# szemenyeim/RoboCupVision

Measured on AMD Instinct MI355X. Metric: training images/sec, ROBO-UNet 640x480 bs=32/GPU, higher is better.
Workload: dtype f32; 1 GPU; robo_unet_640x480_bs32; per_gpu_batch=32, global_batch=32, height=480, width=640, step=fwd+CE/argmax+bwd+L1+Adam (train.py:43-74), parallelism=dp1, launch=eager (one rcv_run per pass)

## Files before the change

include/rcv.h:

```cpp
#ifndef RCV_H
#define RCV_H

#include <stddef.h>
#include <stdint.h>

#ifdef __cplusplus
extern "C" {
#endif

#define RCV_VERSION 100

#define RCV_OK            0
#define RCV_E_ARG        -1
#define RCV_E_HIP        -2
#define RCV_E_UNSUPPORTED -3

typedef struct rcv_handle rcv_handle;

int  rcv_create(int device, rcv_handle** out);
int  rcv_create_planner(int num_cus, rcv_handle** out);
int  rcv_destroy(rcv_handle* h);
const char* rcv_last_error(void);
int  rcv_version(void);
int  rcv_num_cus(const rcv_handle* h);
// ... 29 lines not shown
  RCV_OP_SGD         = 27,
  RCV_OP_NOP         = 28,
  RCV_OP_WGRAD_REDUCE_BATCH = 29,
  RCV_OP_POOL_CLS_FWD = 30,
  RCV_OP_POOL_CLS_BWD = 31,
  RCV_OP_OBJECT_MATCH = 32,
  RCV_OP_LP_TAIL_FWD = 33,
  RCV_OP_LP_TAIL_BWD = 34,
  RCV_OP_LP_BATCH = 35,
  RCV_OP_BATCH_PREP = 36,
  RCV_OP_CLS_LABEL = 37,
  RCV_OP_FRAME_PREP = 38,
  RCV_OP_BNN_STAGE_FWD = 39,
  RCV_OP_BNN_STAGE_BWD = 40,
  RCV_OP_BNN_HEAD_FWD = 41,
  RCV_OP_BNN_HEAD_BWD = 42
};

enum {
  RCV_LOAD_PLAIN    = 0,
  RCV_LOAD_AFFINE   = 1,
  RCV_LOAD_GRAD_ENC = 2,
  RCV_LOAD_GRAD_DEC = 3,
  RCV_LOAD_NCHW     = 4,
  RCV_LOAD_AFFINE_RELU = 5
};

enum {
  RCV_STATS_NONE   = 0,
  RCV_STATS_FWD    = 1,
  RCV_STATS_BWD_ENC= 2,
// ... 173 lines not shown
```

robocupvision_amd/_lib.py:

```python
from __future__ import annotations

import ctypes as C
import os
import threading

_HERE = os.path.dirname(os.path.abspath(__file__))
LIB_PATH = os.environ.get("RCV_LIBRARY") or os.path.join(_HERE, "librcv.so")

RCV_I_N, RCV_I_H, RCV_I_W, RCV_I_CIN, RCV_I_COUT, RCV_I_HO, RCV_I_WO, RCV_I_STRIDE, RCV_I_DIL, \
    RCV_I_INMODE, RCV_I_INMODE2, RCV_I_STATS, RCV_I_NPART, RCV_I_NSPLIT, RCV_I_COUNT, RCV_I_AUX0, RCV_I_AUX1 = range(17)
RCV_I__N = 20
(RCV_P_IN, RCV_P_IN_AUX, RCV_P_IN_C, RCV_P_W, RCV_P_BIAS, RCV_P_OUT, RCV_P_RESID, RCV_P_EPI_AUX, RCV_P_EPI_C,
 RCV_P_PART, RCV_P_IN2, RCV_P_IN2_AUX, RCV_P_IN2_C, RCV_P_X0, RCV_P_X1, RCV_P_X2, RCV_P_X3, RCV_P_X4, RCV_P_X5) = range(19)
RCV_P__N = 20

(OP_CONV, OP_TCONV, OP_WGRAD, OP_WGRAD_REDUCE, OP_PACK, OP_BN_FINALIZE, OP_BN_EVAL, OP_BN_BWD, OP_COMBINE, OP_CLS_FWD,
 OP_CLS_BWD, OP_CE_FWD, OP_CE_BWD, OP_POOL_FWD, OP_POOL_BWD, OP_ADAM_L1, OP_MEMSET, OP_CONV1X1, OP_ADD_SLICE,
 OP_MATERIALIZE, OP_BWD_STATS, OP_CONFUSION, OP_DICE_FWD, OP_DICE_BWD, OP_NHWC_TO_NCHW, OP_NCHW_TO_NHWC, OP_SGD, OP_NOP,
 OP_WGRAD_REDUCE_BATCH, OP_POOL_CLS_FWD, OP_POOL_CLS_BWD) = range(1, 32)
OP_OBJECT_MATCH = 32
OP_LP_TAIL_FWD, OP_LP_TAIL_BWD, OP_LP_BATCH = 33, 34, 35
OP_BATCH_PREP = 36
OP_CLS_LABEL = 37
OP_FRAME_PREP = 38
OP_BNN_STAGE_FWD, OP_BNN_STAGE_BWD, OP_BNN_HEAD_FWD, OP_BNN_HEAD_BWD = 39, 40, 41, 42
CLS_LABEL_FEATURES, CLS_LABEL_LOGITS, CLS_LABEL_CLASSMAP = range(3)

LOAD_PLAIN, LOAD_AFFINE, LOAD_GRAD_ENC, LOAD_GRAD_DEC, LOAD_NCHW, LOAD_AFFINE_RELU = range(6)
STATS_NONE, STATS_FWD, STATS_BWD_ENC, STATS_BWD_DEC = range(4)
F_BIAS, F_RELU, F_RESID, F_OUT_NCHW, F_FLIP, F_TRANSPOSED_SRC, F_ARGMAX, F_TRAINING, F_CONCAT = 1, 2, 4, 8, 16, 32, 64, 128, 256
F_FUSED_UP = 512
F_FUSED_CE = 1024
F_SIDE_STREAM = 1 << 16
F_MFMA_FP32 = 1 << 17


class RcvOp(C.Structure):
    _fields_ = [("kind", C.c_int32), ("flags", C.c_uint32), ("i", C.c_int32 * RCV_I__N), ("f", C.c_float * 8),
                ("p", C.c_void_p * RCV_P__N)]

# ... 161 lines not shown
```

robocupvision_amd/csrc/small_kernels.hip:

```cpp
#include "rcv_internal.h"
#include "cls_common.h"

__device__ __forceinline__ float wave_sum(float v) {
#pragma unroll
  for (int sh = 32; sh >= 1; sh >>= 1) v += __shfl_xor(v, sh);
  return v;
}
__device__ __forceinline__ double wave_sum_d(double v) {
#pragma unroll
  for (int sh = 32; sh >= 1; sh >>= 1) v += __shfl_xor(v, sh);
  return v;
}

__global__ void pack_kernel(const rcv_pack_job* __restrict__ jobs) {
  const rcv_pack_job jb = jobs[blockIdx.y];
  const int per_tap = jb.rows_pad * jb.cols_pad;
  if (jb.merged == 2) {
    const int rows = jb.rows_from_d1 ? jb.D1 : jb.D0;
    const int cols = jb.rows_from_d1 ? jb.D0 : jb.D1;
    for (int e = blockIdx.x * blockDim.x + threadIdx.x; e < per_tap; e += gridDim.x * blockDim.x) {
      const int row = e / jb.cols_pad, col = e - row * jb.cols_pad;
      float g[3][3];
      const bool ok = row < rows && col < cols;
      const int d0 = jb.rows_from_d1 ? col : row, d1 = jb.rows_from_d1 ? row : col;
// ... 185 lines not shown
    v.x = fmaxf(fmaf(a.x, s.x, h.x), 0.f); v.y = fmaxf(fmaf(a.y, s.y, h.y), 0.f);
    v.z = fmaxf(fmaf(a.z, s.z, h.z), 0.f); v.w = fmaxf(fmaf(a.w, s.w, h.w), 0.f);
    float4 b = sld4(r + e * 4);
    if (mode2 != RCV_LOAD_PLAIN) {
      const float4 s2 = sld4(rc + ch), h2 = sld4(rc + C + ch);
      b.x = fmaf(b.x, s2.x, h2.x); b.y = fmaf(b.y, s2.y, h2.y); b.z = fmaf(b.z, s2.z, h2.z); b.w = fmaf(b.w, s2.w, h2.w);
      if (mode2 == RCV_LOAD_AFFINE_RELU) { b.x = fmaxf(b.x, 0.f); b.y = fmaxf(b.y, 0.f); b.z = fmaxf(b.z, 0.f); b.w = fmaxf(b.w, 0.f); }
    }
    sst4(out + pix * 2 * C + ch, v);
    sst4(out + pix * 2 * C + C + ch, b);
  }
}

#define CE_MAX_C 8

template <int CIN, bool FUSED, bool CE>
__global__ void cls_fwd_kernel(const float* __restrict__ x, const float* __restrict__ w, const float* __restrict__ bias,
                               float* __restrict__ out, int N, int HW, int COUT, const float* __restrict__ tc,
                               const float* __restrict__ r, const float* __restrict__ rc, int mode2,
                               const int64_t* __restrict__ target, const float* __restrict__ cw, float* __restrict__ part,
                               uint8_t* __restrict__ argmax, int rch) {
  __shared__ float ws[CLS_MAX_OUT * CIN + CLS_MAX_OUT];
  __shared__ double sh[3][4];
  for (int e = threadIdx.x; e < COUT * CIN; e += blockDim.x) ws[e] = w[e];
  for (int e = threadIdx.x; e < COUT; e += blockDim.x) ws[CLS_MAX_OUT * CIN + e] = bias ? bias[e] : 0.f;
  __syncthreads();
  double a_nll = 0.0, a_w = 0.0, a_ok = 0.0;
  const size_t total = (size_t)N * HW;
  for (size_t p = (size_t)blockIdx.x * blockDim.x + threadIdx.x; p < total; p += (size_t)gridDim.x * blockDim.x) {
    float v[CIN];
    cls_load_up<CIN, FUSED>(v, x, tc, r, rc, mode2, p, rch);
    const size_t n = p / HW, hw = p % HW;
    float lg[CLS_MAX_OUT];
#pragma unroll
    for (int c = 0; c < CLS_MAX_OUT; ++c) {
      if (c < COUT) {
        float u = ws[CLS_MAX_OUT * CIN + c];
#pragma unroll
        for (int k = 0; k < CIN; ++k) u = fmaf(v[k], ws[c * CIN + k], u);
        __builtin_nontemporal_store(u, out + (n * COUT + c) * HW + hw);
        lg[c] = u;
      }
    }
    if (CE) {
      float mx = -INFINITY;
      int am = 0;
#pragma unroll
      for (int c = 0; c < CLS_MAX_OUT; ++c) if (c < COUT && lg[c] > mx) { mx = lg[c]; am = c; }
      float se = 0.f;
#pragma unroll
      for (int c = 0; c < CLS_MAX_OUT; ++c) if (c < COUT) se += expf(lg[c] - mx);
      const int tg = (int)target[p];
      float vt = 0.f;
#pragma unroll
      for (int c = 0; c < CLS_MAX_OUT; ++c) if (c == tg && c < COUT) vt = lg[c];
      const float wt = (unsigned)tg < (unsigned)COUT ? (cw ? cw[tg] : 1.f) : 0.f;
      const float nll = (mx - vt) + logf(se);
      a_nll += (double)(wt * nll);
      a_w += (double)wt;
      a_ok += (am == tg) ? 1.0 : 0.0;
      if (argmax) argmax[p] = (uint8_t)am;
    }
  }
  if (CE) {
    a_nll = wave_sum_d(a_nll); a_w = wave_sum_d(a_w); a_ok = wave_sum_d(a_ok);
    const int wv = threadIdx.x >> 6;
    if ((threadIdx.x & 63) == 0) { sh[0][wv] = a_nll; sh[1][wv] = a_w; sh[2][wv] = a_ok; }
    __syncthreads();
    if (threadIdx.x < 3) {
      double t = 0.0;
      for (int i = 0; i < (int)(blockDim.x >> 6); ++i) t += sh[threadIdx.x][i];
      part[(size_t)blockIdx.x * 3 + threadIdx.x] = (float)t;
    }
  }
}

template <bool FUSED>
__global__ __launch_bounds__(256) void cls_fwd16_kernel(const float* __restrict__ x, const float* __restrict__ w, const float* __restrict__ bias,
                                                        float* __restrict__ out, int N, int HW, int COUT, const float* __restrict__ tc,
                                                        const float* __restrict__ r, const float* __restrict__ rc, int mode2, int rch) {
  constexpr int CIN = 16;
  __shared__ float ws[CLS_MAX_OUT * CIN + CLS_MAX_OUT];
  for (int e = threadIdx.x; e < CLS_MAX_OUT * CIN; e += blockDim.x) ws[e] = e < COUT * CIN ? w[e] : 0.f;
  for (int e = threadIdx.x; e < CLS_MAX_OUT; e += blockDim.x) ws[CLS_MAX_OUT * CIN + e] = (bias && e < COUT) ? bias[e] : 0.f;
  __syncthreads();
  const int q = threadIdx.x & 3;
  float4 s = make_float4(1.f, 1.f, 1.f, 1.f), h = make_float4(0.f, 0.f, 0.f, 0.f), s2 = s, h2 = h;
  if (FUSED) {
// ... 20 lines not shown
#pragma unroll
    for (int c = 0; c < CLS_MAX_OUT; ++c) {
      const float* wc = ws + c * CIN + 4 * q;
      float u = fmaf(a.x, wc[0], fmaf(a.y, wc[1], fmaf(a.z, wc[2], a.w * wc[3])));
      u += __shfl_xor(u, 1);
      u += __shfl_xor(u, 2);
      lg[c] = u + ws[CLS_MAX_OUT * CIN + c];
    }
    const size_t n = p / HW, hw = p % HW;
#pragma unroll
    for (int c = 0; c < CLS_MAX_OUT; ++c)
      if ((c & 3) == q && c < COUT) out[(n * COUT + c) * HW + hw] = lg[c];
  }
}

template <int CIN, int COUT, bool FUSED, bool CE>
__global__ __launch_bounds__(256, (CIN == 8 ? 2 : 1)) void cls_bwd_kernel(const float* __restrict__ up, const float* __restrict__ dl, const float* __restrict__ w,
                               float* __restrict__ dup, const float* __restrict__ t, const float* __restrict__ tc,
                               float* __restrict__ stat_part, float* __restrict__ w_part, int N, int HW, int stats,
                               const float* __restrict__ r, const float* __restrict__ rc, int mode2,
                               const int64_t* __restrict__ target, const float* __restrict__ cw, const float* __restrict__ bias,
                               const float* __restrict__ loss_out, const float* __restrict__ grad_out) {
  __shared__ float ws[COUT * CIN];
  __shared__ float red[4][COUT * CIN + COUT + 2 * CIN];
  for (int e = threadIdx.x; e < COUT * CIN; e += blockDim.x) ws[e] = w[e];
  __syncthreads();
  float dw[COUT][CIN], db[COUT], s1[CIN], s2[CIN];
#pragma unroll
  for (int c = 0; c < COUT; ++c) { db[c] = 0.f;
#pragma unroll
    for (int k = 0; k < CIN; ++k) dw[c][k] = 0.f; }
#pragma unroll
  for (int k = 0; k < CIN; ++k) { s1[k] = 0.f; s2[k] = 0.f; }
  const size_t total = (size_t)N * HW;
  const size_t stride = (size_t)gridDim.x * blockDim.x;
  size_t p = (size_t)blockIdx.x * blockDim.x + threadIdx.x;
  ClsRaw<CIN, FUSED> cur;
  int64_t tcur = 0;
  if (p < total) { cls_load_raw<CIN, FUSED>(cur, FUSED ? t : up, r, p); if (CE) tcur = target[p]; }
  for (; p < total; p += stride) {
    const size_t pn = p + stride < total ? p + stride : p;
    ClsRaw<CIN, FUSED> nxt;
    cls_load_raw<CIN, FUSED>(nxt, FUSED ? t : up, r, pn);
    int64_t tnxt = 0;
    if (CE) tnxt = target[pn];
    const size_t n = p / HW, hw = p % HW;
    float g[COUT], u[CIN], d[CIN];
    cls_form_up<CIN, FUSED>(u, cur, tc, rc, mode2);
    if (CE) {
      float mx = -INFINITY;
#pragma unroll
      for (int c = 0; c < COUT; ++c) {
        float lgc = bias ? bias[c] : 0.f;
#pragma unroll
        for (int k = 0; k < CIN; ++k) lgc = fmaf(u[k], ws[c * CIN + k], lgc);
        g[c] = lgc;
        mx = fmaxf(mx, lgc);
      }
      float se = 0.f;
#pragma unroll
      for (int c = 0; c < COUT; ++c) { g[c] = expf(g[c] - mx); se += g[c]; }
      const int tg = (int)tcur;
      const float kf = (grad_out[0] / loss_out[1]) * ((unsigned)tg < (unsigned)COUT ? (cw ? cw[tg] : 1.f) : 0.f);
      const float inv = 1.f / se;
#pragma unroll
      for (int c = 0; c < COUT; ++c) g[c] = __fmul_rn(kf, fmaf(g[c], inv, c == tg ? -1.f : 0.f));
    } else {
#pragma unroll
      for (int c = 0; c < COUT; ++c) g[c] = dl[(n * COUT + c) * HW + hw];
    }
#pragma unroll
    for (int k = 0; k < CIN; ++k) {
      float acc = 0.f;
#pragma unroll
      for (int c = 0; c < COUT; ++c) acc = fmaf(g[c], ws[c * CIN + k], acc);
      d[k] = acc;
    }
    if (CIN == 8 && (total & 63) == 0) {
      const int lane = threadIdx.x & 63;
      const size_t wave_p0 = p - lane;
#pragma unroll
      for (int sidx = 0; sidx < 2; ++sidx) {
        const int src = sidx * 32 + (lane >> 1);
        float4 lo, hi;
        lo.x = __shfl(d[0], src); lo.y = __shfl(d[1], src); lo.z = __shfl(d[2], src); lo.w = __shfl(d[3], src);
        hi.x = __shfl(d[4], src); hi.y = __shfl(d[5], src); hi.z = __shfl(d[6], src); hi.w = __shfl(d[7], src);
        sst4(dup + (wave_p0 + sidx * 32) * CIN + lane * 4, (lane & 1) ? hi : lo);
      }
    } else {
#pragma unroll
      for (int q = 0; q < CIN / 4; ++q) sst4(dup + p * CIN + 4 * q, make_float4(d[4 * q], d[4 * q + 1], d[4 * q + 2], d[4 * q + 3]));
    }
#pragma unroll
    for (int c = 0; c < COUT; ++c) {
      db[c] += g[c];
#pragma unroll
      for (int k = 0; k < CIN; ++k) dw[c][k] = fmaf(g[c], u[k], dw[c][k]);
    }
    if (stats == RCV_STATS_BWD_DEC) {
#pragma unroll
      for (int q = 0; q < CIN / 4; ++q) {
        const float4 a = FUSED ? cur.a[q] : sld4(t + p * CIN + 4 * q);
// ... 18 lines not shown
    if (lane == 0) red[wv][COUT * CIN + c] = v;
  }
#pragma unroll
  for (int k = 0; k < CIN; ++k) {
    const float v1 = wave_sum(s1[k]), v2 = wave_sum(s2[k]);
    if (lane == 0) { red[wv][COUT * CIN + COUT + k] = v1; red[wv][COUT * CIN + COUT + CIN + k] = v2; }
  }
  __syncthreads();
  const int nw = blockDim.x >> 6;
  for (int e = threadIdx.x; e < COUT * CIN + COUT + 2 * CIN; e += blockDim.x) {
    float v = 0.f;
    for (int i = 0; i < nw; ++i) v += red[i][e];
    if (e < COUT * CIN + COUT) w_part[(size_t)blockIdx.x * (COUT * CIN + COUT) + e] = v;
    else if (stats == RCV_STATS_BWD_DEC) stat_part[(size_t)blockIdx.x * 2 * CIN + (e - COUT * CIN - COUT)] = v;
  }
}

__global__ void rows_reduce_kernel(const float* __restrict__ part, int n_rows, int width, float* __restrict__ out0, int n0,
                                   float* __restrict__ out1) {
  const int e = blockIdx.x;
  double s = 0.0, dummy = 0.0;
  for (int i = threadIdx.x; i < n_rows; i += blockDim.x) s += (double)part[(size_t)i * width + e];
  block_sum2_d(s, dummy);
  if (threadIdx.x == 0) {
    if (e < n0) out0[e] = (float)s;
    else if (out1) out1[e - n0] = (float)s;
  }
}

__global__ void ce_fwd_kernel(const float* __restrict__ logits, const int64_t* __restrict__ target, const float* __restrict__ cw,
                              int N, int C, int HW, float* __restrict__ part, uint8_t* __restrict__ argmax) {
  __shared__ double sh[3][4];
  double a_nll = 0.0, a_w = 0.0, a_ok = 0.0;
  const size_t total = (size_t)N * HW;
  for (size_t p = (size_t)blockIdx.x * blockDim.x + threadIdx.x; p < total; p += (size_t)gridDim.x * blockDim.x) {
    const size_t n = p / HW, hw = p % HW;
    float v[CE_MAX_C];
    float mx = -INFINITY;
    int am = 0;
#pragma unroll
    for (int c = 0; c < CE_MAX_C; ++c) {
      if (c < C) {
// ... 14 lines not shown
    a_w += (double)w;
    a_ok += (am == tg) ? 1.0 : 0.0;
    if (argmax) argmax[p] = (uint8_t)am;
  }
  a_nll = wave_sum_d(a_nll); a_w = wave_sum_d(a_w); a_ok = wave_sum_d(a_ok);
  const int wv = threadIdx.x >> 6;
  if ((threadIdx.x & 63) == 0) { sh[0][wv] = a_nll; sh[1][wv] = a_w; sh[2][wv] = a_ok; }
  __syncthreads();
  if (threadIdx.x < 3) {
    double s = 0.0;
    for (int i = 0; i < (int)(blockDim.x >> 6); ++i) s += sh[threadIdx.x][i];
    part[(size_t)blockIdx.x * 3 + threadIdx.x] = (float)s;
  }
}

__global__ void ce_finalize_kernel(const float* __restrict__ part, int n_part, float* __restrict__ loss_out) {
  __shared__ double sh[3][4];
  double s[3] = {0.0, 0.0, 0.0};
  for (int i = threadIdx.x; i < n_part; i += blockDim.x) {
    s[0] += (double)part[(size_t)i * 3 + 0]; s[1] += (double)part[(size_t)i * 3 + 1]; s[2] += (double)part[(size_t)i * 3 + 2];
  }
  const int wv = threadIdx.x >> 6;
  for (int j = 0; j < 3; ++j) { s[j] = wave_sum_d(s[j]); if ((threadIdx.x & 63) == 0) sh[j][wv] = s[j]; }
  __syncthreads();
  if (threadIdx.x == 0) {
    double t[3] = {0.0, 0.0, 0.0};
    for (int j = 0; j < 3; ++j) for (int i = 0; i < (int)(blockDim.x >> 6); ++i) t[j] += sh[j][i];
    loss_out[0] = (float)(t[0] / t[1]);
    loss_out[1] = (float)t[1];
    loss_out[2] = (float)t[2];
    loss_out[3] = (float)t[0];
  }
}

__global__ void ce_bwd_kernel(const float* __restrict__ logits, const int64_t* __restrict__ target, const float* __restrict__ cw,
                              const float* __restrict__ loss_out, const float* __restrict__ grad_out, int N, int C, int HW,
                              float* __restrict__ dlogits) {
  const float scale = grad_out[0] / loss_out[1];
  const size_t total = (size_t)N * HW;
  for (size_t p = (size_t)blockIdx.x * blockDim.x + threadIdx.x; p < total; p += (size_t)gridDim.x * blockDim.x) {
    const size_t n = p / HW, hw = p % HW;
    float v[CE_MAX_C];
    float mx = -INFINITY;
#pragma unroll
    for (int c = 0; c < CE_MAX_C; ++c) if (c < C) { v[c] = logits[(n * C + c) * HW + hw]; mx = fmaxf(mx, v[c]); }
    float se = 0.f;
#pragma unroll
// ... 510 lines not shown
template <int CIN, bool FUSED, bool CE>
static cls_bwd_fn cls_bwd_pick(int cout) {
  switch (cout) {
    case 1: return cls_bwd_kernel<CIN, 1, FUSED, CE>;
    case 2: return cls_bwd_kernel<CIN, 2, FUSED, CE>;
    case 3: return cls_bwd_kernel<CIN, 3, FUSED, CE>;
    case 4: return cls_bwd_kernel<CIN, 4, FUSED, CE>;
    case 5: return cls_bwd_kernel<CIN, 5, FUSED, CE>;
    case 6: return cls_bwd_kernel<CIN, 6, FUSED, CE>;
    case 7: return cls_bwd_kernel<CIN, 7, FUSED, CE>;
    case 8: return cls_bwd_kernel<CIN, 8, FUSED, CE>;
  }
  return nullptr;
}

int rcv_launch_small(const rcv_handle* h, const rcv_op* op, hipStream_t s, OpQuery* query) {
  const int N = op->i[RCV_I_N], H = op->i[RCV_I_H], W = op->i[RCV_I_W];
  const int Cin = op->i[RCV_I_CIN], Cout = op->i[RCV_I_COUT];
  if (query) {
    static const char* names[] = {"?", "conv", "tconv", "wgrad", "wgrad_reduce", "pack", "bn_finalize", "bn_eval", "bn_bwd", "combine",
                                  "cls_fwd", "cls_bwd", "ce_fwd", "ce_bwd", "pool_fwd", "pool_bwd", "adam_l1", "memset", "conv1x1",
                                  "add_slice", "materialize", "bwd_stats", "confusion", "dice_fwd", "dice_bwd", "nhwc_to_nchw",
                                  "nchw_to_nhwc", "sgd"};
    query->n_part = 0; query->n_split = 0; query->part_bytes = 0;
    snprintf(query->label, sizeof(query->label), "%s", (op->kind > 0 && op->kind <= 27) ? names[op->kind] : "?");
  }
  switch (op->kind) {
    case RCV_OP_PACK: {
      if (query) return RCV_OK;
      const int count = op->i[RCV_I_COUNT], max_elems = op->i[RCV_I_AUX0];
// ... 127 lines not shown
        dl = nullptr;
      } else if (fused) {
        RCV_CHECK_ARG(r && (mode2 == RCV_LOAD_PLAIN || rc), "classifier backward (fused decoder output): operands missing");
        kern = cls_bwd_pick<8, true, false>(Cout);
      } else {
        kern = Cin == 8 ? cls_bwd_pick<8, false, false>(Cout) : cls_bwd_pick<16, false, false>(Cout);
      }
      hipLaunchKernelGGL(kern, dim3(g), dim3(256), 0, s, (const float*)op->p[RCV_P_IN], dl, (const float*)op->p[RCV_P_W], (float*)op->p[RCV_P_OUT],
                         (const float*)op->p[RCV_P_EPI_AUX], (const float*)op->p[RCV_P_EPI_C], stat_part, w_part, N, H * W, stats, r, rc, mode2, tgt,
                         cw, bias, loss_out, grad_out);
      RCV_HIP(hipGetLastError());
      hipLaunchKernelGGL(rows_reduce_kernel, dim3((int)wrow), dim3(256), 0, s, w_part, g, (int)wrow, (float*)op->p[RCV_P_X1], Cout * Cin,
                         (float*)op->p[RCV_P_X2]);
      break;
    }
    case RCV_OP_CE_FWD: {
      const int HW = H * W;
      const int g = reduce_grid(h, (size_t)N * HW, 256);
      RCV_CHECK_ARG(Cout >= 1 && Cout <= CE_MAX_C, "cross entropy: %d classes unsupported (max %d)", Cout, CE_MAX_C);
      if (query) { query->n_part = g; query->part_bytes = (size_t)g * 3 * sizeof(float); return RCV_OK; }
      RCV_CHECK_ARG(op->p[RCV_P_IN] && op->p[RCV_P_IN2] && op->p[RCV_P_PART] && op->p[RCV_P_OUT], "cross entropy: null operand");
      RCV_CHECK_ARG(op->i[RCV_I_NPART] == g, "cross entropy: workspace rows %d != %d", op->i[RCV_I_NPART], g);
      hipLaunchKernelGGL(ce_fwd_kernel, dim3(g), dim3(256), 0, s, (const float*)op->p[RCV_P_IN], (const int64_t*)op->p[RCV_P_IN2],
                         (const float*)op->p[RCV_P_W], N, Cout, HW, (float*)op->p[RCV_P_PART],
                         (op->flags & RCV_F_ARGMAX) ? (uint8_t*)op->p[RCV_P_X0] : nullptr);
      RCV_HIP(hipGetLastError());
      hipLaunchKernelGGL(ce_finalize_kernel, dim3(1), dim3(256), 0, s, (const float*)op->p[RCV_P_PART], g, (float*)op->p[RCV_P_OUT]);
      break;
    }
    case RCV_OP_CE_BWD: {
// ... 208 lines not shown
```

robocupvision_amd/engine.py:

```python
from __future__ import annotations

import collections
import ctypes as C
import os
from typing import Dict, List, Optional, Sequence

import torch

from . import _lib as L

BN_EPS = 1e-5
BN_MOMENTUM = 0.1
SIDE_STREAM_WGRAD = not os.environ.get("RCV_NO_SIDE_STREAM")
SIDE_STREAM_MODE = os.environ.get("RCV_SIDE_STREAM", "auto")
FUSE_UP_INTO_CLS = not os.environ.get("RCV_NO_FUSED_UP")
REDUCE_BATCH = min(int(os.environ.get("RCV_REDUCE_BATCH", "6")), 24)
REDUCE_BATCH_SINGLE = min(int(os.environ.get("RCV_REDUCE_BATCH", "24")), 24)
EVAL_FOLD_BN = not os.environ.get("RCV_NO_EVAL_FOLD")
CLS3_PAD = 8
DGRAD_FIRST = bool(os.environ.get("RCV_DGRAD_FIRST"))
MERGED_TCONV_MAX_COUT = 16
WINOGRAD = os.environ.get("RCV_WINOGRAD", "auto")


# ... 1071 lines not shown
        elif k == L.OP_WGRAD_REDUCE:
            nbytes = 4.0 * i[L.RCV_I_NSPLIT] * (9 * _round_up(cout, 16) * max(_round_up(cin, 4), 4)) + 4.0 * 9 * cin * cout
        elif k == L.OP_WGRAD_REDUCE_BATCH:
            nbytes = 1024.0 * i[L.RCV_I_AUX0]
        elif k in (L.OP_BN_FINALIZE, L.OP_BN_BWD):
            nbytes = 4.0 * i[L.RCV_I_NPART] * 2 * cout
        elif k in (L.OP_CLS_FWD, L.OP_LP_TAIL_FWD):
            flops = 2.0 * cin * cout * px
            skip_c = (i[L.RCV_I_AUX1] or cin) if op.flags & L.F_FUSED_UP else 0
            nbytes = 4.0 * px * (cin + skip_c + cout) + (px * 9.0 if op.flags & L.F_FUSED_CE else 0.0)
        elif k in (L.OP_CLS_BWD, L.OP_LP_TAIL_BWD):
            flops = 2.0 * 2 * cin * cout * px
            rch = i[L.RCV_I_AUX1] if op.flags & L.F_FUSED_UP else 0
            src = cin + ((rch or cin) if op.flags & L.F_FUSED_UP else 0)
            nbytes = 4.0 * px * (src + cin + rch + (0 if op.flags & L.F_FUSED_CE else cout)) + (px * 8.0 if op.flags & L.F_FUSED_CE else 0.0)
        elif k in (L.OP_CE_FWD, L.OP_DICE_FWD):
            nbytes = px * (4.0 * cout + 8 + 1)
        elif k in (L.OP_CE_BWD, L.OP_DICE_BWD):
            nbytes = px * (8.0 * cout + 8)
        elif k == L.OP_POOL_FWD:
            nbytes = 4.0 * px * cout * 1.25
        elif k == L.OP_POOL_BWD:
            nbytes = 4.0 * px * cout * (0.25 + 1 + 1 + resid)
        elif k == L.OP_COMBINE:
            nbytes = 4.0 * px * cout * (2 + (2 if op.flags & L.F_CONCAT else 1))
        elif k == L.OP_MATERIALIZE:
            nbytes = 4.0 * px * cout * 2
        elif k == L.OP_ADD_SLICE:
            nbytes = 4.0 * px * cin * 3
        elif k == L.OP_BWD_STATS:
# ... 7 lines not shown
            nbytes = 4.0 * (px * cin * (1 + reads_r + resid) + n * ho * wo * (2 * cin + cout))
        elif k in (L.OP_NHWC_TO_NCHW, L.OP_NCHW_TO_NHWC):
            nbytes = 4.0 * px * (cin + cout)
        elif k in (L.OP_ADAM_L1, L.OP_SGD):
            nbytes = 4.0 * (i[L.RCV_I_COUNT] & 0xFFFFFFFF) * (7 if k == L.OP_ADAM_L1 else 5)
        elif k == L.OP_MEMSET:
            nbytes = 4.0 * i[L.RCV_I_COUNT]
        elif k == L.OP_PACK:
            nbytes = 8.0 * i[L.RCV_I_AUX0] * 0
        return flops, nbytes

    def profile_last(self, reps: int = 3, with_loss: bool = True):
        plan, _inputs = self._last
        stream = torch.cuda.current_stream(self.device).cuda_stream
        ce = plan.ce if (with_loss and plan.ce) else None
        lists = [ce["fwd"] if ce else plan.fwd]
        bwd = ce["bwd"] if ce else plan.bwd
        if bwd is not None and bwd.n:
            if not ce:
                dl = torch.full_like(plan.logits, 1e-4)
                for (idx, slot) in plan.dlogits_slots:
                    plan.bwd.arr[idx].p[slot] = dl.data_ptr()
            lists.append(bwd)
        rows = []
        for lst in lists:
            labels = lst.labels(self.handle)
            acc = [0.0] * lst.n
            for _ in range(reps):
                for k, v in enumerate(lst.run_timed(self.handle, stream)):
                    acc[k] += v
# ... 46 lines not shown
            ms = []
            for mode in self.SIDE_MODES:
                self._set_side(ops, mode)
                ops.run(self.handle, stream.cuda_stream)
                e0, e1 = torch.cuda.Event(enable_timing=True), torch.cuda.Event(enable_timing=True)
                e0.record(stream)
                for _ in range(3):
                    ops.run(self.handle, stream.cuda_stream)
                e1.record(stream)
                e1.synchronize()
                ms.append(e0.elapsed_time(e1) / 3)
            plan.side_ms = tuple(ms)
            best = min(range(len(ms)), key=lambda k: ms[k])
            plan.side_mode = self.SIDE_MODES[best if ms[best] < 0.97 * ms[0] else 0]
        plan.side_on = plan.side_mode != "off"
        for lst in (plan.bwd, plan.ce["bwd"] if plan.ce else None):
            if lst is not None:
                self._set_side(lst, plan.side_mode)

    def _run_backward(self, plan: Plan, ops):
        if self.dry_run:
            plan.side_decided = True
            stream = 0
        else:
            if not plan.side_decided:
                self._decide_side_stream(plan, ops)
            stream = torch.cuda.current_stream(self.device).cuda_stream
        if self.grad_ready_cb is None or not plan.bwd_marks:
            ops.run(self.handle, stream)
            return
        run_bucketed(plan.bwd_marks, self.flat.numel, self.grad_buckets, ops.n,
# ... 18 lines not shown
        loss_out = self._zeros(plan, 4)
        argmax = self._alloc(plan, N, H, W, dtype=torch.uint8)
        gone = torch.ones(1, dtype=torch.float32, device=self.device)
        plan.keep.append(gone)
        f.flags |= L.F_FUSED_CE
        f.p[L.RCV_P_X1] = loss_out.data_ptr()
        f.p[L.RCV_P_X2] = argmax.data_ptr()
        self._workspace(plan, f)
        b.flags |= L.F_FUSED_CE
        b.p[L.RCV_P_BIAS] = f.p[L.RCV_P_BIAS]
        b.p[L.RCV_P_X5] = loss_out.data_ptr()
        b.p[L.RCV_P_IN2_AUX] = gone.data_ptr()
        plan.ce = {"fwd": L.OpList(fops), "bwd": L.OpList(bops), "kf": kf[0], "kb": kb[0], "loss_out": loss_out, "argmax": argmax}
        plan.ce["fwd"].labels(self.handle)
        plan.ce["bwd"].labels(self.handle)
        return plan.ce

    def forward_ce(self, inputs: Sequence[torch.Tensor], targets: torch.Tensor, weight: Optional[torch.Tensor]):
        for t in inputs:
            if t.dtype != torch.float32 or not t.is_contiguous():
                raise L.RcvError("engine inputs must be contiguous float32 tensors")
        plan = self._plan_for(inputs, True)
        ce = self._ce_variant(plan)
        if ce is None:
            return None
        N, H, W = ce["argmax"].shape
        if targets.dtype != torch.int64 or not targets.is_contiguous() or tuple(targets.shape) != (N, H, W) or targets.device != self.device:
            raise L.RcvError("targets must be a contiguous int64 [B,H,W] tensor on the model's device")
        for k, t in enumerate(inputs):
            for (is_bwd, idx, slot) in plan.input_slots[k]:
                (ce["bwd"] if is_bwd else ce["fwd"]).arr[idx].p[slot] = t.data_ptr()
                (plan.bwd if is_bwd else plan.fwd).arr[idx].p[slot] = t.data_ptr()
        wptr = None if weight is None else weight.data_ptr()
        for op in (ce["fwd"].arr[ce["kf"]], ce["bwd"].arr[ce["kb"]]):
            op.p[L.RCV_P_IN2] = targets.data_ptr()
            op.p[L.RCV_P_X0] = wptr
        ce["fwd"].run(self.handle, torch.cuda.current_stream(self.device).cuda_stream)
        self.params_dirty = True
        nbt = [m.num_batches_tracked for m in self.bn_modules if m.num_batches_tracked is not None]
        if nbt:
            torch._foreach_add_(nbt, 1)
        self._last = (plan, [t for t in inputs])
        self._generation += 1
        self._last_ce = (targets, weight)
        return plan.logits, ce["loss_out"], ce["argmax"]

    def backward_ce(self):
        plan, _inputs = self._last
        self._run_backward(plan, plan.ce["bwd"])
        return plan
```

robocupvision_amd/train.py:

```python
from __future__ import annotations

import os
from typing import Optional, Sequence

import torch

from . import _lib as L
from .model import CrossEntropyLoss2d, DiceLoss, LabelProp
from .optim import AdamL1


class _HipStreams:

    def __init__(self, device, overlap: bool):
        self.device = device
        self.comm = torch.cuda.Stream(device=device) if overlap else None

    def current(self):
        return torch.cuda.current_stream(self.device)

    def wait(self, waiter, waited):
        waiter.wait_stream(waited)

    def ptr(self, stream) -> int:
# ... 48 lines not shown
        dev = next(model.parameters()).device
        if dev.type != "cuda":
            raise L.RcvError("Trainer needs the model on the HIP device (model.cuda())")
        self.device = dev
        w = None if class_weights is None else torch.tensor(list(class_weights), dtype=torch.float32, device=dev)
        if use_dice:
            if w is None:
                raise ValueError("DiceLoss needs class weights")
            self.criterion = DiceLoss(w).to(dev)
        else:
            self.criterion = CrossEntropyLoss2d(w).to(dev)
        self.optimizer = optimizer if optimizer is not None else AdamL1(model, lr=lr, decay=decay, transfer=transfer)
        self.metrics = torch.zeros(4, dtype=torch.float64, device=dev)
        self.distributed = distributed
        self.fuse_loss = fuse_loss and not os.environ.get("RCV_NO_FUSED_LOSS")
        self.world = 1
        self.exchange: Optional[GradExchange] = None
        self.force_collectives = bool(int(os.environ.get("RCV_FORCE_COLLECTIVES", "0")))
        self.prune_indices = None
        if prune_indices is not None:
            self.set_prune_indices(prune_indices)
        if distributed:
            if getattr(model, "classify", False):
                raise L.RcvError("data-parallel training of the patch-classification mode (classify) is not built; train it on one GPU "
                                 "with a stock loss and optimizer (classTrainer.py)")
            import torch.distributed as dist
            if not dist.is_initialized():
                raise L.RcvError("distributed=True needs torch.distributed.init_process_group('nccl') first")
            self.world = dist.get_world_size()
            self.optimizer.grad_scale = 1.0 / self.world
# ... 20 lines not shown
        model, opt, crit = self.model, self.optimizer, self.criterion
        model.train()
        opt.zero_grad(set_to_none=True)
        eng = model._get_engine()
        exchanging = self.exchange is not None and (self.world > 1 or self.force_collectives)
        eng.grad_ready_cb = self.exchange.grad_ready if exchanging else None
        if exchanging:
            self.exchange.begin()
        fused = None
        ins = model._engine_inputs(imgs) if hasattr(model, "_engine_inputs") else [imgs]
        if self.fuse_loss and type(crit) is CrossEntropyLoss2d and ins[0].dtype == torch.float32 and ins[0].is_contiguous():
            w = crit.weight
            if w is not None and w.device != imgs.device:
                w = w.to(imgs.device)
                crit.weight = w
            fused = eng.forward_ce(ins, targets.to(torch.int64).contiguous(), w)
        if fused is not None:
            pred, out, argmax = fused
            crit.last_stats, crit.last_argmax = out, argmax
            ce = out[0]
            eng.backward_ce()
            fl = eng.flat
            for k, p in enumerate(fl.params):
                if eng.param_used[k]:
                    p.grad = fl.grad_view(k)
        else:
            pred = model(imgs)
            ce = crit(pred, targets)
            ce.backward()
        if exchanging:
            self.exchange.finish()
# ... 68 lines not shown
```

Baseline: 5926 img/s.

## Fuse classifier forward, cross-entropy and classifier backward into one training-step kernel

Replaces the separate classifier forward (with CE/argmax) and classifier backward passes with a single kernel that computes logits, writes them and the argmax, accumulates CE partials and computes gradients in one sweep over the activations. A small ce_norm kernel computes the class-weight normaliser ahead of time so the backward scale is known before the loss is finalised. A combined tail kernel reduces the weight gradients and finalises the loss together. This removes one full read of the 8-channel input features and the logits, plus a few kernel launches. The cost is an extra pass over the targets and more register pressure in the fused kernel.

```diff
diff --git a/include/rcv.h b/include/rcv.h
--- a/include/rcv.h
+++ b/include/rcv.h
@@ -67,7 +67,9 @@
   RCV_OP_BNN_STAGE_FWD = 39,
   RCV_OP_BNN_STAGE_BWD = 40,
   RCV_OP_BNN_HEAD_FWD = 41,
-  RCV_OP_BNN_HEAD_BWD = 42
+  RCV_OP_BNN_HEAD_BWD = 42,
+  RCV_OP_CE_NORM = 43,
+  RCV_OP_CLS_STEP = 44
 };
 
 enum {
diff --git a/robocupvision_amd/_lib.py b/robocupvision_amd/_lib.py
--- a/robocupvision_amd/_lib.py
+++ b/robocupvision_amd/_lib.py
@@ -24,6 +24,7 @@
 OP_CLS_LABEL = 37
 OP_FRAME_PREP = 38
 OP_BNN_STAGE_FWD, OP_BNN_STAGE_BWD, OP_BNN_HEAD_FWD, OP_BNN_HEAD_BWD = 39, 40, 41, 42
+OP_CE_NORM, OP_CLS_STEP = 43, 44
 CLS_LABEL_FEATURES, CLS_LABEL_LOGITS, CLS_LABEL_CLASSMAP = range(3)
 
 LOAD_PLAIN, LOAD_AFFINE, LOAD_GRAD_ENC, LOAD_GRAD_DEC, LOAD_NCHW, LOAD_AFFINE_RELU = range(6)
diff --git a/robocupvision_amd/csrc/small_kernels.hip b/robocupvision_amd/csrc/small_kernels.hip
--- a/robocupvision_amd/csrc/small_kernels.hip
+++ b/robocupvision_amd/csrc/small_kernels.hip
@@ -1,5 +1,6 @@
 #include "rcv_internal.h"
 #include "cls_common.h"
+#include <type_traits>
 
 __device__ __forceinline__ float wave_sum(float v) {
 #pragma unroll
@@ -223,6 +224,46 @@
 
 #define CE_MAX_C 8
 
+__device__ __forceinline__ float ce_label_weight(int tg, int C, const float* __restrict__ cw) {
+  return (unsigned)tg < (unsigned)C ? (cw ? cw[tg] : 1.f) : 0.f;
+}
+template <int NC>
+__device__ __forceinline__ float ce_first_max(const float (&lg)[NC], int C, int& am) {
+  float mx = -INFINITY;
+  am = 0;
+#pragma unroll
+  for (int c = 0; c < NC; ++c) if (c < C && lg[c] > mx) { mx = lg[c]; am = c; }
+  return mx;
+}
+template <int NC>
+__device__ __forceinline__ float ce_target_logit(const float (&lg)[NC], int C, int tg) {
+  float vt = 0.f;
+#pragma unroll
+  for (int c = 0; c < NC; ++c) if (c == tg && c < C) vt = lg[c];
+  return vt;
+}
+template <class OK>
+__device__ __forceinline__ void ce_pixel_sums(float mx, float vt, float se, int am, int tg, int C, const float* __restrict__ cw,
+                                              double& a_nll, double& a_w, OK& a_ok) {
+  const float wt = ce_label_weight(tg, C, cw);
+  const float nll = (mx - vt) + logf(se);
+  a_nll += (double)(wt * nll);
+  a_w += (double)wt;
+  a_ok += (am == tg) ? OK(1) : OK(0);
+}
+__device__ __forceinline__ void ce_store_row(double a_nll, double a_w, double a_ok, float* __restrict__ row, const float* __restrict__ w_row = nullptr) {
+  __shared__ double sh[3][4];
+  a_nll = wave_sum_d(a_nll); a_w = wave_sum_d(a_w); a_ok = wave_sum_d(a_ok);
+  const int wv = threadIdx.x >> 6;
+  if ((threadIdx.x & 63) == 0) { sh[0][wv] = a_nll; sh[1][wv] = a_w; sh[2][wv] = a_ok; }
+  __syncthreads();
+  if (threadIdx.x < 3) {
+    double t = 0.0;
+    for (int i = 0; i < (int)(blockDim.x >> 6); ++i) t += sh[threadIdx.x][i];
+    row[threadIdx.x] = (w_row && threadIdx.x == 1) ? w_row[0] : (float)t;
+  }
+}
+
 template <int CIN, bool FUSED, bool CE>
 __global__ void cls_fwd_kernel(const float* __restrict__ x, const float* __restrict__ w, const float* __restrict__ bias,
                                float* __restrict__ out, int N, int HW, int COUT, const float* __restrict__ tc,
@@ -230,7 +271,6 @@
                                const int64_t* __restrict__ target, const float* __restrict__ cw, float* __restrict__ part,
                                uint8_t* __restrict__ argmax, int rch) {
   __shared__ float ws[CLS_MAX_OUT * CIN + CLS_MAX_OUT];
-  __shared__ double sh[3][4];
   for (int e = threadIdx.x; e < COUT * CIN; e += blockDim.x) ws[e] = w[e];
   for (int e = threadIdx.x; e < COUT; e += blockDim.x) ws[CLS_MAX_OUT * CIN + e] = bias ? bias[e] : 0.f;
   __syncthreads();
@@ -252,35 +292,40 @@
       }
     }
     if (CE) {
-      float mx = -INFINITY;
-      int am = 0;
-#pragma unroll
-      for (int c = 0; c < CLS_MAX_OUT; ++c) if (c < COUT && lg[c] > mx) { mx = lg[c]; am = c; }
+      int am;
+      const float mx = ce_first_max(lg, COUT, am);
       float se = 0.f;
 #pragma unroll
       for (int c = 0; c < CLS_MAX_OUT; ++c) if (c < COUT) se += expf(lg[c] - mx);
       const int tg = (int)target[p];
-      float vt = 0.f;
-#pragma unroll
-      for (int c = 0; c < CLS_MAX_OUT; ++c) if (c == tg && c < COUT) vt = lg[c];
-      const float wt = (unsigned)tg < (unsigned)COUT ? (cw ? cw[tg] : 1.f) : 0.f;
-      const float nll = (mx - vt) + logf(se);
-      a_nll += (double)(wt * nll);
-      a_w += (double)wt;
-      a_ok += (am == tg) ? 1.0 : 0.0;
+      ce_pixel_sums(mx, ce_target_logit(lg, COUT, tg), se, am, tg, COUT, cw, a_nll, a_w, a_ok);
       if (argmax) argmax[p] = (uint8_t)am;
     }
   }
-  if (CE) {
-    a_nll = wave_sum_d(a_nll); a_w = wave_sum_d(a_w); a_ok = wave_sum_d(a_ok);
-    const int wv = threadIdx.x >> 6;
-    if ((threadIdx.x & 63) == 0) { sh[0][wv] = a_nll; sh[1][wv] = a_w; sh[2][wv] = a_ok; }
-    __syncthreads();
-    if (threadIdx.x < 3) {
-      double t = 0.0;
-      for (int i = 0; i < (int)(blockDim.x >> 6); ++i) t += sh[threadIdx.x][i];
-      part[(size_t)blockIdx.x * 3 + threadIdx.x] = (float)t;
-    }
+  if (CE) ce_store_row(a_nll, a_w, a_ok, part + (size_t)blockIdx.x * 3);
+}
+
+__global__ void ce_norm_kernel(const int64_t* __restrict__ target, const float* __restrict__ cw, int C, size_t total,
+                               float* __restrict__ rows) {
+  __shared__ double sh[4];
+  double a_w = 0.0;
+  const size_t stride = (size_t)gridDim.x * blockDim.x;
+  size_t p = (size_t)blockIdx.x * blockDim.x + threadIdx.x;
+  for (; p + 3 * stride < total; p += 4 * stride) {
+    const int t0 = (int)target[p], t1 = (int)target[p + stride], t2 = (int)target[p + 2 * stride], t3 = (int)target[p + 3 * stride];
+    a_w += (double)ce_label_weight(t0, C, cw);
+    a_w += (double)ce_label_weight(t1, C, cw);
+    a_w += (double)ce_label_weight(t2, C, cw);
+    a_w += (double)ce_label_weight(t3, C, cw);
+  }
+  for (; p < total; p += stride) a_w += (double)ce_label_weight((int)target[p], C, cw);
+  a_w = wave_sum_d(a_w);
+  if ((threadIdx.x & 63) == 0) sh[threadIdx.x >> 6] = a_w;
+  __syncthreads();
+  if (threadIdx.x == 0) {
+    double t = 0.0;
+    for (int i = 0; i < (int)(blockDim.x >> 6); ++i) t += sh[i];
+    rows[blockIdx.x] = (float)t;
   }
 }
 
@@ -331,17 +376,47 @@
   }
 }
 
-template <int CIN, int COUT, bool FUSED, bool CE>
+struct ClsStepArgs {
+  float* logits;
+  uint8_t* argmax;
+  float* ce_part;
+  const float* norm_rows;
+  int n_rows;
+};
+
+template <class T>
+__device__ __forceinline__ const T& cls_first_arg(const T& a) { return a; }
+
+template <int CIN, int COUT, bool FUSED, bool CE, class... STEP_ARGS>
 __global__ __launch_bounds__(256, (CIN == 8 ? 2 : 1)) void cls_bwd_kernel(const float* __restrict__ up, const float* __restrict__ dl, const float* __restrict__ w,
                                float* __restrict__ dup, const float* __restrict__ t, const float* __restrict__ tc,
                                float* __restrict__ stat_part, float* __restrict__ w_part, int N, int HW, int stats,
                                const float* __restrict__ r, const float* __restrict__ rc, int mode2,
                                const int64_t* __restrict__ target, const float* __restrict__ cw, const float* __restrict__ bias,
-                               const float* __restrict__ loss_out, const float* __restrict__ grad_out) {
+                               const float* __restrict__ loss_out, const float* __restrict__ grad_out, STEP_ARGS... step_args) {
+  constexpr bool STEP = sizeof...(STEP_ARGS) != 0;
+  static_assert(!STEP || (CE && FUSED && CIN == 8), "the training-step form is the fused 8-channel classifier with its loss");
+  [[maybe_unused]] ClsStepArgs sa{};
+  if constexpr (STEP) { sa = cls_first_arg(step_args...); stats = RCV_STATS_BWD_DEC; }
   __shared__ float ws[COUT * CIN];
   __shared__ float red[4][COUT * CIN + COUT + 2 * CIN];
   for (int e = threadIdx.x; e < COUT * CIN; e += blockDim.x) ws[e] = w[e];
-  __syncthreads();
+  float sum_w = 0.f;
+  double a_nll = 0.0, a_w = 0.0;
+  int n_ok = 0;
+  if constexpr (STEP) {
+    __shared__ double shn[4];
+    double sn = 0.0;
+    for (int i = threadIdx.x; i < sa.n_rows; i += blockDim.x) sn += (double)sa.norm_rows[i];
+    sn = wave_sum_d(sn);
+    if ((threadIdx.x & 63) == 0) shn[threadIdx.x >> 6] = sn;
+    __syncthreads();
+    double tn = 0.0;
+    for (int i = 0; i < (int)(blockDim.x >> 6); ++i) tn += shn[i];
+    sum_w = (float)tn;
+  } else {
+    __syncthreads();
+  }
   float dw[COUT][CIN], db[COUT], s1[CIN], s2[CIN];
 #pragma unroll
   for (int c = 0; c < COUT; ++c) { db[c] = 0.f;
@@ -349,18 +424,21 @@
     for (int k = 0; k < CIN; ++k) dw[c][k] = 0.f; }
 #pragma unroll
   for (int k = 0; k < CIN; ++k) { s1[k] = 0.f; s2[k] = 0.f; }
+  float ce_scale = 0.f;
+  if constexpr (STEP) ce_scale = __int_as_float(__builtin_amdgcn_readfirstlane(__float_as_int(grad_out[0] / sum_w)));
+  using label_t = typename std::conditional<STEP, int, int64_t>::type;
   const size_t total = (size_t)N * HW;
   const size_t stride = (size_t)gridDim.x * blockDim.x;
   size_t p = (size_t)blockIdx.x * blockDim.x + threadIdx.x;
   ClsRaw<CIN, FUSED> cur;
-  int64_t tcur = 0;
-  if (p < total) { cls_load_raw<CIN, FUSED>(cur, FUSED ? t : up, r, p); if (CE) tcur = target[p]; }
+  label_t tcur = 0;
+  if (p < total) { cls_load_raw<CIN, FUSED>(cur, FUSED ? t : up, r, p); if (CE) tcur = (label_t)target[p]; }
   for (; p < total; p += stride) {
     const size_t pn = p + stride < total ? p + stride : p;
     ClsRaw<CIN, FUSED> nxt;
     cls_load_raw<CIN, FUSED>(nxt, FUSED ? t : up, r, pn);
-    int64_t tnxt = 0;
-    if (CE) tnxt = target[pn];
+    label_t tnxt = 0;
+    if (CE) tnxt = (label_t)target[pn];
     const size_t n = p / HW, hw = p % HW;
     float g[COUT], u[CIN], d[CIN];
     cls_form_up<CIN, FUSED>(u, cur, tc, rc, mode2);
@@ -371,14 +449,27 @@
         float lgc = bias ? bias[c] : 0.f;
 #pragma unroll
         for (int k = 0; k < CIN; ++k) lgc = fmaf(u[k], ws[c * CIN + k], lgc);
+        if constexpr (STEP) __builtin_nontemporal_store(lgc, sa.logits + (n * COUT + c) * HW + hw);
         g[c] = lgc;
         mx = fmaxf(mx, lgc);
       }
+      const int tg = (int)tcur;
+      int am = 0;
+      float mxf = 0.f, vt = 0.f;
+      if constexpr (STEP) {
+        mxf = ce_first_max(g, COUT, am);
+        vt = ce_target_logit(g, COUT, tg);
+      }
       float se = 0.f;
 #pragma unroll
       for (int c = 0; c < COUT; ++c) { g[c] = expf(g[c] - mx); se += g[c]; }
-      const int tg = (int)tcur;
-      const float kf = (grad_out[0] / loss_out[1]) * ((unsigned)tg < (unsigned)COUT ? (cw ? cw[tg] : 1.f) : 0.f);
+      if constexpr (STEP) {
+        ce_pixel_sums(mxf, vt, se, am, tg, COUT, cw, a_nll, a_w, n_ok);
+        if (sa.argmax) sa.argmax[p] = (uint8_t)am;
+      }
+      float kf;
+      if constexpr (STEP) kf = ce_scale * ce_label_weight(tg, COUT, cw);
+      else kf = (grad_out[0] / loss_out[1]) * ((unsigned)tg < (unsigned)COUT ? (cw ? cw[tg] : 1.f) : 0.f);
       const float inv = 1.f / se;
 #pragma unroll
       for (int c = 0; c < COUT; ++c) g[c] = __fmul_rn(kf, fmaf(g[c], inv, c == tg ? -1.f : 0.f));
@@ -396,13 +487,20 @@
     if (CIN == 8 && (total & 63) == 0) {
       const int lane = threadIdx.x & 63;
       const size_t wave_p0 = p - lane;
+      float* wave_dup = dup + wave_p0 * CIN;
+      if constexpr (STEP) {
+        const uintptr_t wave_v = reinterpret_cast<uintptr_t>(wave_dup);
+        wave_dup = reinterpret_cast<float*>(((uintptr_t)(uint32_t)__builtin_amdgcn_readfirstlane((int)(wave_v >> 32)) << 32) |
+                                            (uint32_t)__builtin_amdgcn_readfirstlane((int)(uint32_t)wave_v));
+      }
 #pragma unroll
       for (int sidx = 0; sidx < 2; ++sidx) {
         const int src = sidx * 32 + (lane >> 1);
         float4 lo, hi;
         lo.x = __shfl(d[0], src); lo.y = __shfl(d[1], src); lo.z = __shfl(d[2], src); lo.w = __shfl(d[3], src);
         hi.x = __shfl(d[4], src); hi.y = __shfl(d[5], src); hi.z = __shfl(d[6], src); hi.w = __shfl(d[7], src);
-        sst4(dup + (wave_p0 + sidx * 32) * CIN + lane * 4, (lane & 1) ? hi : lo);
+        if constexpr (STEP) sst4(wave_dup + sidx * 32 * CIN + lane * 4, (lane & 1) ? hi : lo);
+        else sst4(dup + (wave_p0 + sidx * 32) * CIN + lane * 4, (lane & 1) ? hi : lo);
       }
     } else {
 #pragma unroll
@@ -451,11 +549,11 @@
     if (e < COUT * CIN + COUT) w_part[(size_t)blockIdx.x * (COUT * CIN + COUT) + e] = v;
     else if (stats == RCV_STATS_BWD_DEC) stat_part[(size_t)blockIdx.x * 2 * CIN + (e - COUT * CIN - COUT)] = v;
   }
-}
-
-__global__ void rows_reduce_kernel(const float* __restrict__ part, int n_rows, int width, float* __restrict__ out0, int n0,
-                                   float* __restrict__ out1) {
-  const int e = blockIdx.x;
+  if constexpr (STEP) ce_store_row(a_nll, 0.0, (double)n_ok, sa.ce_part + (size_t)blockIdx.x * 3, sa.norm_rows + blockIdx.x);
+}
+
+__device__ __forceinline__ void rows_reduce_body(const float* __restrict__ part, int n_rows, int width, float* __restrict__ out0, int n0,
+                                                 float* __restrict__ out1, int e) {
   double s = 0.0, dummy = 0.0;
   for (int i = threadIdx.x; i < n_rows; i += blockDim.x) s += (double)part[(size_t)i * width + e];
   block_sum2_d(s, dummy);
@@ -463,6 +561,11 @@
     if (e < n0) out0[e] = (float)s;
     else if (out1) out1[e - n0] = (float)s;
   }
+}
+
+__global__ void rows_reduce_kernel(const float* __restrict__ part, int n_rows, int width, float* __restrict__ out0, int n0,
+                                   float* __restrict__ out1) {
+  rows_reduce_body(part, n_rows, width, out0, n0, out1, blockIdx.x);
 }
 
 __global__ void ce_fwd_kernel(const float* __restrict__ logits, const int64_t* __restrict__ target, const float* __restrict__ cw,
@@ -507,7 +610,7 @@
   }
 }
 
-__global__ void ce_finalize_kernel(const float* __restrict__ part, int n_part, float* __restrict__ loss_out) {
+__device__ __forceinline__ void ce_finalize_body(const float* __restrict__ part, int n_part, float* __restrict__ loss_out) {
   __shared__ double sh[3][4];
   double s[3] = {0.0, 0.0, 0.0};
   for (int i = threadIdx.x; i < n_part; i += blockDim.x) {
@@ -524,6 +627,16 @@
     loss_out[2] = (float)t[2];
     loss_out[3] = (float)t[0];
   }
+}
+
+__global__ void ce_finalize_kernel(const float* __restrict__ part, int n_part, float* __restrict__ loss_out) {
+  ce_finalize_body(part, n_part, loss_out);
+}
+
+__global__ void cls_step_tail_kernel(const float* __restrict__ w_part, int n_rows, int width, float* __restrict__ dw, int n0,
+                                     float* __restrict__ db, const float* __restrict__ ce_part, float* __restrict__ loss_out) {
+  if ((int)blockIdx.x == width) ce_finalize_body(ce_part, n_rows, loss_out);
+  else rows_reduce_body(w_part, n_rows, width, dw, n0, db, blockIdx.x);
 }
 
 __global__ void ce_bwd_kernel(const float* __restrict__ logits, const int64_t* __restrict__ target, const float* __restrict__ cw,
@@ -1064,6 +1177,23 @@
   return nullptr;
 }
 
+typedef void (*cls_step_fn)(const float*, const float*, const float*, float*, const float*, const float*, float*, float*, int, int, int,
+                            const float*, const float*, int, const int64_t*, const float*, const float*, const float*, const float*, ClsStepArgs);
+
+static cls_step_fn cls_step_pick(int cout) {
+  switch (cout) {
+    case 1: return cls_bwd_kernel<8, 1, true, true, ClsStepArgs>;
+    case 2: return cls_bwd_kernel<8, 2, true, true, ClsStepArgs>;
+    case 3: return cls_bwd_kernel<8, 3, true, true, ClsStepArgs>;
+    case 4: return cls_bwd_kernel<8, 4, true, true, ClsStepArgs>;
+    case 5: return cls_bwd_kernel<8, 5, true, true, ClsStepArgs>;
+    case 6: return cls_bwd_kernel<8, 6, true, true, ClsStepArgs>;
+    case 7: return cls_bwd_kernel<8, 7, true, true, ClsStepArgs>;
+    case 8: return cls_bwd_kernel<8, 8, true, true, ClsStepArgs>;
+  }
+  return nullptr;
+}
+
 int rcv_launch_small(const rcv_handle* h, const rcv_op* op, hipStream_t s, OpQuery* query) {
   const int N = op->i[RCV_I_N], H = op->i[RCV_I_H], W = op->i[RCV_I_W];
   const int Cin = op->i[RCV_I_CIN], Cout = op->i[RCV_I_COUT];
@@ -1221,6 +1351,57 @@
                          (float*)op->p[RCV_P_X2]);
       break;
     }
+    case RCV_OP_CE_NORM: {
+      const int g = reduce_grid(h, (size_t)N * H * W, 256);
+      RCV_CHECK_ARG(Cout >= 1 && Cout <= CE_MAX_C, "cross entropy normaliser: %d classes unsupported (max %d)", Cout, CE_MAX_C);
+      RCV_CHECK_ARG(N > 0 && H > 0 && W > 0, "cross entropy normaliser: empty batch");
+      if (query) {
+        snprintf(query->label, sizeof(query->label), "ce_norm");
+        query->n_part = g; query->part_bytes = (size_t)g * sizeof(float);
+        return RCV_OK;
+      }
+      RCV_CHECK_ARG(op->p[RCV_P_IN2] && op->p[RCV_P_PART], "cross entropy normaliser: null operand");
+      RCV_CHECK_ARG(op->i[RCV_I_NPART] == g, "cross entropy normaliser: workspace rows %d != %d", op->i[RCV_I_NPART], g);
+      hipLaunchKernelGGL(ce_norm_kernel, dim3(g), dim3(256), 0, s, (const int64_t*)op->p[RCV_P_IN2], (const float*)op->p[RCV_P_X0], Cout,
+                         (size_t)N * H * W, (float*)op->p[RCV_P_PART]);
+      break;
+    }
+    case RCV_OP_CLS_STEP: {
+      const int g = reduce_grid(h, (size_t)N * H * W, 256);
+      const size_t wrow = (size_t)Cout * Cin + Cout;
+      const int mode2 = op->i[RCV_I_AUX0];
+      RCV_CHECK_ARG(Cin == 8 && Cout >= 1 && Cout <= CLS_MAX_OUT, "classifier step: %d -> %d channels unsupported (8 input channels, 1..%d classes)",
+                    Cin, Cout, CLS_MAX_OUT);
+      RCV_CHECK_ARG((op->flags & RCV_F_FUSED_UP) && (op->flags & RCV_F_FUSED_CE) && op->i[RCV_I_STATS] == RCV_STATS_BWD_DEC,
+                    "classifier step: needs the fused decoder input (RCV_F_FUSED_UP), the fused loss (RCV_F_FUSED_CE) and the decoder's statistics kind");
+      RCV_CHECK_ARG(op->i[RCV_I_AUX1] == 0 || op->i[RCV_I_AUX1] == Cin, "classifier step: %d skip channels for %d inputs", op->i[RCV_I_AUX1], Cin);
+      RCV_CHECK_ARG(mode2 == RCV_LOAD_PLAIN || mode2 == RCV_LOAD_AFFINE || mode2 == RCV_LOAD_AFFINE_RELU, "classifier step: skip load mode %d", mode2);
+      if (query) {
+        snprintf(query->label, sizeof(query->label), "cls_step");
+        query->n_part = g;
+        query->part_bytes = (size_t)g * (2 * Cin + wrow) * sizeof(float);
+        return RCV_OK;
+      }
+      const float* r = (const float*)op->p[RCV_P_X3]; const float* rc = (const float*)op->p[RCV_P_X4];
+      RCV_CHECK_ARG(op->p[RCV_P_EPI_AUX] && op->p[RCV_P_EPI_C] && r && (mode2 == RCV_LOAD_PLAIN || rc) && op->p[RCV_P_W] && op->p[RCV_P_IN2] &&
+                    op->p[RCV_P_IN2_AUX], "classifier step: null input operand");
+      RCV_CHECK_ARG(op->p[RCV_P_OUT] && op->p[RCV_P_RESID] && op->p[RCV_P_PART] && op->p[RCV_P_IN2_C] && op->p[RCV_P_IN_C] && op->p[RCV_P_X1] &&
+                    op->p[RCV_P_X5], "classifier step: null output or workspace operand");
+      RCV_CHECK_ARG(op->i[RCV_I_NPART] == g, "classifier step: workspace rows %d != %d", op->i[RCV_I_NPART], g);
+      float* stat_part = (float*)op->p[RCV_P_PART];
+      float* w_part = stat_part + (size_t)g * 2 * Cin;
+      ClsStepArgs sa;
+      sa.logits = (float*)op->p[RCV_P_RESID]; sa.argmax = (uint8_t*)op->p[RCV_P_IN_AUX]; sa.ce_part = (float*)op->p[RCV_P_IN2_C];
+      sa.norm_rows = (const float*)op->p[RCV_P_IN_C]; sa.n_rows = g;
+      hipLaunchKernelGGL(cls_step_pick(Cout), dim3(g), dim3(256), 0, s, (const float*)nullptr, (const float*)nullptr, (const float*)op->p[RCV_P_W],
+                         (float*)op->p[RCV_P_OUT], (const float*)op->p[RCV_P_EPI_AUX], (const float*)op->p[RCV_P_EPI_C], stat_part, w_part, N, H * W,
+                         (int)RCV_STATS_BWD_DEC, r, rc, mode2, (const int64_t*)op->p[RCV_P_IN2], (const float*)op->p[RCV_P_X0],
+                         (const float*)op->p[RCV_P_BIAS], (const float*)nullptr, (const float*)op->p[RCV_P_IN2_AUX], sa);
+      RCV_HIP(hipGetLastError());
+      hipLaunchKernelGGL(cls_step_tail_kernel, dim3((int)wrow + 1), dim3(256), 0, s, (const float*)w_part, g, (int)wrow, (float*)op->p[RCV_P_X1],
+                         Cout * Cin, (float*)op->p[RCV_P_X2], (const float*)sa.ce_part, (float*)op->p[RCV_P_X5]);
+      break;
+    }
     case RCV_OP_CE_FWD: {
       const int HW = H * W;
       const int g = reduce_grid(h, (size_t)N * HW, 256);
diff --git a/robocupvision_amd/engine.py b/robocupvision_amd/engine.py
--- a/robocupvision_amd/engine.py
+++ b/robocupvision_amd/engine.py
@@ -1109,6 +1109,11 @@
             rch = i[L.RCV_I_AUX1] if op.flags & L.F_FUSED_UP else 0
             src = cin + ((rch or cin) if op.flags & L.F_FUSED_UP else 0)
             nbytes = 4.0 * px * (src + cin + rch + (0 if op.flags & L.F_FUSED_CE else cout)) + (px * 8.0 if op.flags & L.F_FUSED_CE else 0.0)
+        elif k == L.OP_CLS_STEP:
+            flops = 2.0 * 3 * cin * cout * px
+            nbytes = 4.0 * px * (cin + (i[L.RCV_I_AUX1] or cin) + cout + cin) + px * 9.0
+        elif k == L.OP_CE_NORM:
+            nbytes = px * 8.0
         elif k in (L.OP_CE_FWD, L.OP_DICE_FWD):
             nbytes = px * (4.0 * cout + 8 + 1)
         elif k in (L.OP_CE_BWD, L.OP_DICE_BWD):
@@ -1146,6 +1151,8 @@
         plan, _inputs = self._last
         stream = torch.cuda.current_stream(self.device).cuda_stream
         ce = plan.ce if (with_loss and plan.ce) else None
+        if ce:
+            ce = ce.get("ran") or ce
         lists = [ce["fwd"] if ce else plan.fwd]
         bwd = ce["bwd"] if ce else plan.bwd
         if bwd is not None and bwd.n:
@@ -1222,7 +1229,7 @@
             best = min(range(len(ms)), key=lambda k: ms[k])
             plan.side_mode = self.SIDE_MODES[best if ms[best] < 0.97 * ms[0] else 0]
         plan.side_on = plan.side_mode != "off"
-        for lst in (plan.bwd, plan.ce["bwd"] if plan.ce else None):
+        for lst in (plan.bwd, plan.ce["bwd"] if plan.ce else None, plan.ce["step"]["bwd"] if plan.ce and plan.ce["step"] else None):
             if lst is not None:
                 self._set_side(lst, plan.side_mode)
 
@@ -1271,9 +1278,33 @@
         plan.ce = {"fwd": L.OpList(fops), "bwd": L.OpList(bops), "kf": kf[0], "kb": kb[0], "loss_out": loss_out, "argmax": argmax}
         plan.ce["fwd"].labels(self.handle)
         plan.ce["bwd"].labels(self.handle)
+        plan.ce["step"] = self._cls_step_variant(plan, fops, bops, f, b)
         return plan.ce
 
-    def forward_ce(self, inputs: Sequence[torch.Tensor], targets: torch.Tensor, weight: Optional[torch.Tensor]):
+    def _cls_step_variant(self, plan: Plan, fops, bops, f: L.RcvOp, b: L.RcvOp):
+        if f.kind != L.OP_CLS_FWD or b.kind != L.OP_CLS_BWD or (b.flags & L.F_RESID):
+            return None
+        if any((is_bwd, idx) in ((False, len(fops) - 1), (True, 0)) for slots in plan.input_slots for (is_bwd, idx, _slot) in slots):
+            return None
+        if f.i[L.RCV_I_CIN] != 8 or b.i[L.RCV_I_STATS] != L.STATS_BWD_DEC or f.i[L.RCV_I_AUX1] not in (0, 8):
+            return None
+        norm = L.make_op(L.OP_CE_NORM, 0, n=f.i[L.RCV_I_N], h=f.i[L.RCV_I_H], w=f.i[L.RCV_I_W], cout=f.i[L.RCV_I_COUT])
+        self._workspace(plan, norm)
+        st = L.RcvOp.from_buffer_copy(b)
+        st.kind = L.OP_CLS_STEP
+        st.p[L.RCV_P_RESID] = f.p[L.RCV_P_OUT]
+        st.p[L.RCV_P_IN_AUX] = f.p[L.RCV_P_X2]
+        st.p[L.RCV_P_IN2_C] = f.p[L.RCV_P_PART]
+        st.p[L.RCV_P_IN_C] = norm.p[L.RCV_P_PART]
+        if f.i[L.RCV_I_NPART] != st.i[L.RCV_I_NPART] or norm.i[L.RCV_I_NPART] != st.i[L.RCV_I_NPART]:
+            return None
+        sf = L.OpList([L.RcvOp.from_buffer_copy(o) for o in fops[:-1]] + [norm, st])
+        sb = L.OpList([L.make_op(L.OP_NOP, 0)] + [L.RcvOp.from_buffer_copy(o) for o in bops[1:]])
+        sf.labels(self.handle)
+        sb.labels(self.handle)
+        return {"fwd": sf, "bwd": sb, "knorm": sf.n - 2, "kstep": sf.n - 1}
+
+    def forward_ce(self, inputs: Sequence[torch.Tensor], targets: torch.Tensor, weight: Optional[torch.Tensor], step: bool = False):
         for t in inputs:
             if t.dtype != torch.float32 or not t.is_contiguous():
                 raise L.RcvError("engine inputs must be contiguous float32 tensors")
@@ -1289,10 +1320,21 @@
                 (ce["bwd"] if is_bwd else ce["fwd"]).arr[idx].p[slot] = t.data_ptr()
                 (plan.bwd if is_bwd else plan.fwd).arr[idx].p[slot] = t.data_ptr()
         wptr = None if weight is None else weight.data_ptr()
-        for op in (ce["fwd"].arr[ce["kf"]], ce["bwd"].arr[ce["kb"]]):
+        st = ce["step"] if step else None
+        if st:
+            lists = st
+            for k, t in enumerate(inputs):
+                for (is_bwd, idx, slot) in plan.input_slots[k]:
+                    (st["bwd"] if is_bwd else st["fwd"]).arr[idx].p[slot] = t.data_ptr()
+            loss_ops = (st["fwd"].arr[st["knorm"]], st["fwd"].arr[st["kstep"]])
+        else:
+            lists = ce
+            loss_ops = (ce["fwd"].arr[ce["kf"]], ce["bwd"].arr[ce["kb"]])
+        for op in loss_ops:
             op.p[L.RCV_P_IN2] = targets.data_ptr()
             op.p[L.RCV_P_X0] = wptr
-        ce["fwd"].run(self.handle, torch.cuda.current_stream(self.device).cuda_stream)
+        ce["ran"] = lists
+        lists["fwd"].run(self.handle, torch.cuda.current_stream(self.device).cuda_stream)
         self.params_dirty = True
         nbt = [m.num_batches_tracked for m in self.bn_modules if m.num_batches_tracked is not None]
         if nbt:
@@ -1304,5 +1346,5 @@
 
     def backward_ce(self):
         plan, _inputs = self._last
-        self._run_backward(plan, plan.ce["bwd"])
+        self._run_backward(plan, plan.ce["ran"]["bwd"])
         return plan
diff --git a/robocupvision_amd/train.py b/robocupvision_amd/train.py
--- a/robocupvision_amd/train.py
+++ b/robocupvision_amd/train.py
@@ -86,6 +86,7 @@
         self.metrics = torch.zeros(4, dtype=torch.float64, device=dev)
         self.distributed = distributed
         self.fuse_loss = fuse_loss and not os.environ.get("RCV_NO_FUSED_LOSS")
+        self.fuse_cls_step = not os.environ.get("RCV_NO_FUSED_CLS_STEP")
         self.world = 1
         self.exchange: Optional[GradExchange] = None
         self.force_collectives = bool(int(os.environ.get("RCV_FORCE_COLLECTIVES", "0")))
@@ -136,7 +137,7 @@
             if w is not None and w.device != imgs.device:
                 w = w.to(imgs.device)
                 crit.weight = w
-            fused = eng.forward_ce(ins, targets.to(torch.int64).contiguous(), w)
+            fused = eng.forward_ce(ins, targets.to(torch.int64).contiguous(), w, step=self.fuse_cls_step)
         if fused is not None:
             pred, out, argmax = fused
             crit.last_stats, crit.last_argmax = out, argmax
```

Measured after the change: 6025 img/s (median of 6 runs). +1.7%, better.
